# jordi-adell/mcarray

Hardware: AMD Instinct MI355X
Metric: STFT frames/sec, 8-mic GCC-PHAT + SRP-PHAT(361) + delay-and-sum beamform @48kHz/1024-pt (higher is better)
Workload: dtype f32 (SRP operands adaptive); 1 GPU; BASELINE configs[2] geometry (8-mic ULA 0.04 m, 48 kHz, N=1024, hop 512, 361 angles, 1 source, no power floor), 8 arrays x 4096 frames per GPU per step; channel rows padded by 64 floats; arrays_per_gpu=8, frames_per_array=4096, srp_precision=adaptive, parallelism=arrays sharded over 1 GPU(s), all_gather of DOA bins+prob

## Files before the change

### __graft_entry__.py

```python
import os
import subprocess
import sys

ROOT = os.path.dirname(os.path.abspath(__file__))
if ROOT not in sys.path:
    sys.path.insert(0, ROOT)


def build():
    env = dict(os.environ)
    subprocess.check_call(["make", "-C", os.path.join(ROOT, "mcarray_amd", "csrc"), "-j4", "-s"], env=env)
    subprocess.check_call(["make", "-C", os.path.join(ROOT, "oracle"), "-s"], env=env)
    cxx = os.path.join(ROOT, "tests", "cxx", "Makefile")
    if os.path.exists(cxx):
        subprocess.check_call(["make", "-C", os.path.dirname(cxx), "-s"], env=env)
    harness = os.path.join(ROOT, "tests", "cxx", "gemm_harness.mk")
    if os.path.exists(harness):
        subprocess.check_call(["make", "-C", os.path.dirname(harness), "-f", "gemm_harness.mk", "-s"], env=env)
    import mcarray_amd
    from mcarray_amd import _lib
    _lib.load()


def smoke():
    import numpy as np
    from mcarray_amd import api, synth
    from oracle import pyoracle as po
    fs, N, F = 48000, 1024, 12
    xs = synth.ULA8
    pcm = synth.noise_source_stream(xs, np.deg2rad(23.0), fs, (F + 1) * N // 2, 42)
    ctx = api.Context(fs, xs, N, 0.5, 1, srp_precision=api.SRP_FP32, device=0)
    r = ctx.process_frames_host(pcm[None], want_energy=True)
    o = po.ssl_stream(fs, N, xs, pcm.astype(np.float64), 1, 0.5, want_map=True)
    assert np.array_equal(r["bin"][0], o["bin"]), (r["bin"][0].T, o["bin"].T)
    assert np.abs(r["energy"][0] - o["energy"]).max() <= 2e-5 * np.abs(o["energy"]).max()
    assert np.abs(r["out"][0] - o["out"]).max() <= 2e-5 * np.abs(o["out"]).max() + 1e-7
    print("smoke ok: DOA bins", r["bin"][0, :, 0].tolist(), "->", float(np.rad2deg(r["doa"][0, -1, 0])), "deg")


if __name__ == "__main__":
    build()
    if len(sys.argv) > 1 and sys.argv[1] == "smoke":
        smoke()
```

### mcarray_amd/csrc/kernels_wave.hip

```cpp
#include <type_traits>

#include "fft1024c.h"
#include "mca_internal.h"
#include "cand_unit.h"
#include "phat_pairs.h"
#include "pair_balance.h"
#include "steer.h"
#include "stream_plan.h"

namespace mca {

__global__ __launch_bounds__(256) void k_bf_table(float2 *tab, const float *grid, const double *mic_x, int M, int n_pairs, double unit)
{
    const int d = blockIdx.x, pr = blockIdx.y;
    const double doa = d == 0 ? 0.0 : (double)grid[d - 1];
    const double cd = cos(doa + 1.57079632679489661923);
    const double sc = 1.0 / ((double)M * 1024.0);
    float2 *row = tab + ((long long)d * n_pairs + pr) * 1024;
    for (int k = threadIdx.x; k < 1024; k += 256) {
        const int kap = k <= 512 ? k : k - 1024;
        double pa[2] = {0.0, 0.0}, pb[2] = {0.0, 0.0};
        for (int e = 0; e < 2; ++e) {
            const int c = 2 * pr + e;
            if (c >= M) continue;
// ... 379 lines not shown
        auto load_pair = [&](int f, int pr) {
            const float *pa = base + (long long)(2 * pr) * mstride + (long long)(fr0 + f) * FFT_H;
            const float *pb = pa + mstride;
#pragma unroll
            for (int i = 0; i < 16; ++i) { xa[i] = pa[lofs + 64 * i]; xb[i] = pb[lofs + 64 * i]; }
        };
        const int nfr = f_end - f_begin;
        const int rot = p.list ? 0 : (int)((unsigned)(5 * a + 3 * ((int)blockIdx.x * nw + wave)) % (unsigned)nfr);
        auto frame_of = [&](int i) { const int j = i + rot; return f_begin + (j >= nfr ? j - nfr : j); };
        load_pair(frame_of(0), 0);
        const float4 *srow = nullptr; const float *snyq = nullptr;
        float2 *Yl = buf + F1K_SCRATCH + lam;
        float2 *Qs = wbase + nw * regw + wave * STEER_QWORDS;
        if (FUSE) {
            const int pred = __builtin_amdgcn_readfirstlane(p.bf.pred[a]) + 1;
            srow = p.bf.rows + (long long)pred * (NP * 64);
            snyq = p.bf.nyq + pred * MT;
            if (lane < STEER_QWORDS) Qs[lane] = p.bf.q[(pred * MT + 2 * (lane / 14) + (lane & 1)) * 8 + (lane % 14) / 2 + 1];
            wave_lds_fence();
        }
        for (int fi = 0; fi < nfr; ++fi) {
            const int f = frame_of(fi);
            float2 Xh[MT][8], zn[NP];
            float2 *yrow = FUSE ? p.bf.Y + ((long long)a * p.total_frames + p.frame0 + f) * STEER_ROW : nullptr;
            v2f ptime = {0.f, 0.f};
            bool any_alive = false;
#pragma unroll
            for (int pr = 0; pr < NP; ++pr) {
                float2 z[16];
                if (p.hist_out) {
                    const int j = p.frame0 + f - (p.total_frames - HIST_FRAMES);
                    if (j >= 0) {
                        float *ha = p.hist_out + ((long long)a * MT + 2 * pr) * HIST_SAMPLES + j * FFT_H + (FUSE ? 0 : lane);
#pragma unroll
                        for (int i = 0; i < 8; ++i) { ha[lofs + 64 * i] = xa[i]; ha[lofs + HIST_SAMPLES + 64 * i] = xb[i]; }
                        if (j == HIST_FRAMES - 1) {
#pragma unroll
                            for (int i = 0; i < 8; ++i) { ha[lofs + FFT_H + 64 * i] = xa[8 + i]; ha[lofs + HIST_SAMPLES + FFT_H + 64 * i] = xb[8 + i]; }
                        }
                    }
                }
#pragma unroll
                for (int i = 0; i < 8; ++i) { z[2 * i] = win_lo(xa[2 * i], xb[2 * i], win[i]); z[2 * i + 1] = win_hi(xa[2 * i + 1], xb[2 * i + 1], win[i]); }
                if (POWER) {
#pragma unroll
                    for (int i = 0; i < 16; ++i) { const v2f zv = to_v2f(z[i]); asm("v_pk_fma_f32 %0, %1, %1, %0" : "+v"(ptime) : "v"(zv)); }
                }
                float ma = max3abs(z[0].x, z[1].x, z[2].x), mb = max3abs(z[0].y, z[1].y, z[2].y);
#pragma unroll
                for (int i = 3; i < 15; i += 2) { ma = max3abs(ma, z[i].x, z[i + 1].x); mb = max3abs(mb, z[i].y, z[i + 1].y); }
                ma = max2abs(ma, z[15].x); mb = max2abs(mb, z[15].y);
                const PairBalance pb = pair_balance(ma, mb);
                const bool alive_a = pb.alive_a, alive_b = pb.alive_b;
                any_alive = any_alive || alive_a || alive_b;
                if (pb.scaled()) {
                    const float sa = pb.sa(), sb = pb.sb();
#pragma unroll
                    for (int i = 0; i < 16; ++i) z[i] = make_float2(z[i].x * sa, z[i].y * sb);
                }
                const float4 Bl = FUSE ? (srow + pr * 64)[(unsigned)lane] : make_float4(0.f, 0.f, 0.f, 0.f);
                fft1024c<false, 3>(z, buf, lane, tab, lc, [&]() {
                    const bool lastp = pr == NP - 1, last = lastp && fi + 1 >= nfr;
                    if (FUSE) { Yl[64 * STEER_Y_BASE] = make_float2(Bl.x, Bl.y); Yl[64 * (STEER_Y_BASE + 1)] = make_float2(Bl.z, Bl.w); }
                    load_pair(last ? f : (lastp ? frame_of(fi + 1) : f), last ? pr : (lastp ? 0 : pr + 1));
                }, lam);
                const float un_a = pb.un_a(), un_b = pb.un_b();
                if (MERGE && !FUSE) zn[pr] = make_float2(z[dr16(8)].x * un_a, z[dr16(8)].y * un_b);
                if (FUSE) { const float2 n = make_float2(z[dr16(8)].x * un_a, z[dr16(8)].y * un_b); if (pr < NP - 1) Yl[64 * (STEER_Y_ZN + pr)] = n; else zn[pr] = n; }
                if (lane == 0) {
                    const float2 n = z[dr16(8)];
                    if (!MERGE) nyq[(f - f_begin) * NP + pr] = make_float2(n.x * un_a, n.y * un_b);
                    float2 t[16];
#pragma unroll
                    for (int j = 0; j < 16; ++j) t[j] = z[dr16(j)];
#pragma unroll
                    for (int j = 8; j < 16; ++j) z[dr16(j < 12 ? j + 4 : j - 4)] = t[(j + 1) & 15];
                } else if (self) {
#pragma unroll
                    for (int j = 8; j < 12; ++j) { const float2 t = z[dr16(j)]; z[dr16(j)] = z[dr16(j + 4)]; z[dr16(j + 4)] = t; }
                } else {
#pragma unroll
                    for (int j = 8; j < 12; ++j) {
                        float2 &u = z[dr16(j)], &w = z[dr16(j + 4)];
                        swap_rows32(u.x, w.x); swap_rows32(w.x, u.x);
                        swap_rows32(u.y, w.y); swap_rows32(w.y, u.y);
                    }
                }
                const float thr_a = PairBalance::thr(4e-30f, pb.na, alive_a), thr_b = PairBalance::thr(4e-30f, pb.nb, alive_b);
                const float half_a = PairBalance::down(0.5f, pb.na, alive_a), half_b = PairBalance::down(0.5f, pb.nb, alive_b);
                float4 Bu = make_float4(0.f, 0.f, 0.f, 0.f);
                if (FUSE) { const float2 ba = Yl[64 * STEER_Y_BASE], bb = Yl[64 * (STEER_Y_BASE + 1)]; Bu = steer_base(make_float4(ba.x, ba.y, bb.x, bb.y), un_a, un_b); }
#pragma unroll
                for (int s = 0; s < 8; ++s) {
                    const float2 zk = z[dr16(s)], zm = z[dr16(15 - s < 12 ? 15 - s + 4 : 15 - s - 4)];
                    float2 a2, b2;
                    mirror_split(zk, zm, a2, b2);
                    if constexpr (ULA) whiten4_pair<NOPHAT>(a2, b2, Xh[2 * pr][s], Xh[2 * pr + 1][s], thr_a, thr_b, half_a, half_b);
                    else {
                        float pwa, pwb;
                        Xh[2 * pr][s] = whiten4<NOPHAT>(a2, pwa, thr_a, half_a);
                        Xh[2 * pr + 1][s] = whiten4<NOPHAT>(b2, pwb, thr_b, half_b);
                    }
                    if (FUSE) {
                        float2 y = pr == 0 ? make_float2(0.f, 0.f) : Yl[64 * s];
                        if (s == 0) y = steer_mac<true>(y, a2, b2, Bu, a2, b2);
                        else { const float4 qq = reinterpret_cast<const float4 *>(Qs)[pr * 7 + s - 1]; y = steer_mac<false>(y, a2, b2, Bu, make_float2(qq.x, qq.y), make_float2(qq.z, qq.w)); }
                        if (pr < NP - 1) Yl[64 * s] = y;
                        else yrow[(unsigned)lam + 64 * s] = s == 0 ? steer_dc(y, lane) : y;
                    }
                }
            }
            if (FUSE) {
#pragma unroll
                for (int pr = 0; pr < NP - 1; ++pr) zn[pr] = Yl[64 * (STEER_Y_ZN + pr)];
            }
            if (FUSE && lane == 0) yrow[FFT_H] = make_float2(steer_nyquist<NP>(zn, snyq), 0.f);
            if (p.dead && lane == 0) p.dead[(long long)a * p.total_frames + p.frame0 + f] = any_alive ? 0 : 1;
            OutT *arow = reinterpret_cast<OutT *>(p.A) + (row_base + f) * (long long)p.a_row_elems;
            if (MERGE) {
                float2 *S = buf;
                for (int j = lane; j < nmp / 2; j += 64) reinterpret_cast<float4 *>(S)[j] = make_float4(0.f, 0.f, 0.f, 0.f);
                wave_lds_fence();
                float xn[MT];
#pragma unroll
                for (int pr = 0; pr < NP; ++pr) {
                    float pw;
                    xn[2 * pr] = whiten4(make_float2(2.f * zn[pr].x, 0.f), pw).x;
                    xn[2 * pr + 1] = whiten4(make_float2(2.f * zn[pr].y, 0.f), pw).x;
                }
                const uint2 *offt = reinterpret_cast<const uint2 *>(rankl) + lane;
#pragma unroll
                for (int g = 1; g < MT; ++g) {
#pragma unroll
                    for (int h = 0; h < 2; ++h) {
                        const uint2 o4 = offt[(2 * (g - 1) + h) * 64];
                        const unsigned off[4] = {o4.x & 0xffffu, o4.x >> 16, o4.y & 0xffffu, o4.y >> 16};
                        float2 acc[4], cur[4];
#pragma unroll
                        for (int s2 = 0; s2 < 4; ++s2) {
                            acc[s2] = make_float2(0.f, 0.f);
#pragma unroll
                            for (int i = 0; i + g < MT; ++i) acc[s2] = cmacc(acc[s2], Xh[i][4 * h + s2], Xh[i + g][4 * h + s2]);
                        }
#pragma unroll
                        for (int s2 = 0; s2 < 4; ++s2) cur[s2] = S[off[s2]];
#pragma unroll
                        for (int s2 = 0; s2 < 4; ++s2) S[off[s2]] = cadd(cur[s2], acc[s2]);
                    }
                }
                if (lane == 0) {
                    float an[MT - 1], cn[MT - 1];
                    unsigned on[MT - 1];
#pragma unroll
                    for (int g = 1; g < MT; ++g) {
                        an[g - 1] = 0.f;
#pragma unroll
                        for (int i = 0; i + g < MT; ++i) an[g - 1] = fmaf(xn[i], xn[i + g], an[g - 1]);
                        on[g - 1] = rankl[2 * (MT - 1) * 64 * 4 + g - 1];
                    }
#pragma unroll
                    for (int g = 0; g < MT - 1; ++g) cn[g] = S[on[g]].x;
#pragma unroll
                    for (int g = 0; g < MT - 1; ++g) S[on[g]].x = cn[g] + an[g];
                }
                wave_lds_fence();
                typedef _Float16 half4_t __attribute__((ext_vector_type(4)));
                typedef float float4_t __attribute__((ext_vector_type(4)));
                if (p.planar) {
                    for (int j = lane; j < nmp / 4; j += 64) {
                        const float4 v0 = reinterpret_cast<const float4 *>(S)[2 * j], v1 = reinterpret_cast<const float4 *>(S)[2 * j + 1];
                        const float4_t re = {v0.x, v0.z, v1.x, v1.z}, im = {v0.y, v0.w, v1.y, v1.w};
                        reinterpret_cast<half4_t *>(arow)[j] = __builtin_convertvector(re, half4_t);
                        reinterpret_cast<half4_t *>(arow + nmp)[j] = __builtin_convertvector(im, half4_t);
                    }
                } else
                for (int j = lane; j < nmp / 2; j += 64) {
                    const float4 v = reinterpret_cast<const float4 *>(S)[j];
                    const float4_t vv = {v.x, v.y, v.z, v.w};
                    reinterpret_cast<half4_t *>(arow)[j] = __builtin_convertvector(vv, half4_t);
                }
                wave_lds_fence();
            } else {
#pragma unroll
                for (int s = 0; s < 8; ++s) {
                    if constexpr (ULA) {
                        float2 r[MT], out[NOUT];
#pragma unroll
                        for (int m = 0; m < MT; ++m) r[m] = Xh[m][s];
                        pair_products<MT, ULA>(r, out);
#pragma unroll
                        for (int g = 0; g < NOUT; ++g) store_a_wave<PL2>(arow, voff, g * KG + 64 * s, out[g], p.Kp);
                    } else {
                        int pi = 0;
#pragma unroll
                        for (int i = 0; i < MT; ++i)
#pragma unroll
                            for (int j = i + 1; j < MT; ++j) { store_a_wave<PL2>(arow, voff, pi * KG + 64 * s, cmulc(Xh[i][s], Xh[j][s]), p.Kp); ++pi; }
                    }
                }
            }
            if (POWER) {
                const float pacc = wave_sum64(ptime.x + ptime.y);
                if (lane == 0) p.power[(long long)a * p.total_frames + p.frame0 + f] = pacc / (float)FFT_N / (float)MT;
            }
        }
        wave_lds_fence();
        if (!MERGE && lane < f_end - f_begin) {
            float2 xn[MT], out[NOUT];
#pragma unroll
            for (int pr = 0; pr < NP; ++pr) {
                const float2 n = nyq[lane * NP + pr];
                float pw;
                xn[2 * pr] = whiten4<NOPHAT>(make_float2(2.f * n.x, 0.f), pw);
                xn[2 * pr + 1] = whiten4<NOPHAT>(make_float2(2.f * n.y, 0.f), pw);
            }
            OutT *arow = reinterpret_cast<OutT *>(p.A) + (row_base + f_begin + lane) * (long long)p.a_row_elems;
            pair_products<MT, ULA>(xn, out);
#pragma unroll
            for (int g = 0; g < NOUT; ++g) store_a_wave<PL2>(arow, 0u, g * KG + FFT_H, out[g], p.Kp);
        }
        }
        wave_lds_fence();
        if constexpr (CAND) {
            static_assert(!CAND || PL2, "the candidate contraction reads the two-plane rows of the list mode");
            {
                __syncthreads();
                cand_unit<4>(p.cand, li - p.list0, e_unit, reinterpret_cast<unsigned char *>(wbase), tid);
            }
        }
    }
}

__global__ __launch_bounds__(64) void k_steer_table(float4 *rows, float2 *q, float *nyq, const float *grid, const double *mic_x, int M, double unit)
{
    const int d = blockIdx.x, pr = blockIdx.y, lane = threadIdx.x, lam = lane <= 32 ? lane : 96 - lane;
    const double doa = d == 0 ? 0.0 : (double)grid[d - 1];
    const double cd = cos(doa + 1.57079632679489661923);
    const double sc = 1.0 / ((double)M * 1024.0);
    auto phasor = [&](int c, int k, double &cs, double &sn) {
        double turns = (double)k * (unit * mic_x[c] * cd);
        turns -= rint(turns);
        sincospi(2.0 * turns, &sn, &cs);
    };
    double ca, sa, cb, sb;
    phasor(2 * pr, lam, ca, sa); phasor(2 * pr + 1, lam, cb, sb);
    rows[((long long)d * gridDim.y + pr) * 64 + lane] = make_float4((float)(ca * sc), (float)(sa * sc), (float)(cb * sc), (float)(sb * sc));
    if (lane < 16) {
        const int c = 2 * pr + (lane >> 3), s = lane & 7;
        double cs, sn;
        phasor(c, 64 * s, cs, sn);
        q[((long long)d * M + c) * 8 + s] = make_float2((float)cs, (float)sn);
    }
    if (lane < 2) {
        double cs, sn;
        phasor(2 * pr + lane, 512, cs, sn);
        nyq[d * M + 2 * pr + lane] = (float)(cs * sc);
    }
}

__global__ __launch_bounds__(256, 2) void k_steer_patch(SteerPatchArgs p)
{
    extern __shared__ __attribute__((aligned(16))) unsigned char smem_raw[];
    float2 *tab = reinterpret_cast<float2 *>(smem_raw);
    const int tid = threadIdx.x, lane = tid & 63, wave = __builtin_amdgcn_readfirstlane(tid >> 6);
    float2 *buf = tab + F1K_TWORDS + wave * F1K_SCRATCH;
    const int npass = p.f1 - p.f0, stride = 4 * (int)gridDim.x;
    int work = p.all;
    if (!work) {
        const int first = (int)blockIdx.x * 4 + wave;
        const int per = first < npass ? (npass - first + stride - 1) / stride : 0, items = per * p.n_arrays;
        for (int i = lane; i < items; i += 64) {
            const int a = i / per, fo = first + stride * (i - a * per);
            work |= p.doa_bin[(long long)a * p.n_frames + p.f0 + fo] != p.bf.pred[a];
        }
    }
    if (!__syncthreads_or(work)) return;
    f1k_table_init(tab, tid, 256);
    F1kLane lc;
    lc.init(lane);
    __syncthreads();
    v2f win[8];
#pragma unroll
    for (int i = 0; i < 8; ++i) { win[i].x = p.window[lane + 128 * i]; win[i].y = p.window[lane + 128 * i + 64]; }
    for (int a = 0; a < p.n_arrays; ++a) {
        const int pred = __builtin_amdgcn_readfirstlane(p.bf.pred[a]);
        const bool every = p.all != 0;
        int missed = 0;
        for (int fo = (int)blockIdx.x * 4 + wave; fo < npass; fo += stride) {
            const int f = p.f0 + fo;
            const int bin = __builtin_amdgcn_readfirstlane(p.doa_bin[(long long)a * p.n_frames + f]);
            if (bin != pred) ++missed;
            else if (!every) continue;
            steer_patch_frame(p, a, f, bin, win, buf, tab, lc, lane);
        }
        if (missed && lane == 0) { atomicAdd(p.miss, (unsigned long long)missed); if (pred >= 0) atomicAdd(p.miss + 1, (unsigned long long)missed); }
    }
}

__global__ __launch_bounds__(256) void k_steer_synth(SteerSynthArgs p)
{
    extern __shared__ __attribute__((aligned(16))) unsigned char smem_raw[];
    float2 *tab = reinterpret_cast<float2 *>(smem_raw);
    const int tid = threadIdx.x, lane = tid & 63, wave = __builtin_amdgcn_readfirstlane(tid >> 6);
    float2 *buf = tab + F1K_TWORDS + wave * F1K_SCRATCH;
    f1k_table_init(tab, tid, 256);
    F1kLane lc;
    lc.init(lane);
    __syncthreads();
    const int a = blockIdx.y;
    if (p.pred_out && blockIdx.x == 0 && tid == 0) p.pred_out[a] = p.doa_bin[(long long)a * p.n_frames + p.n_frames - 1];
    if (p.report && blockIdx.x == 0 && a == 0 && tid == 0) {
        const unsigned long long tot = p.miss_total[1];
        p.report[0] = tot - p.miss_total[2];
        p.miss_total[2] = tot;
        __hip_atomic_store(&p.report[1], p.seq, __ATOMIC_RELEASE, __HIP_MEMORY_SCOPE_SYSTEM);
    }
    if (p.n_miss && blockIdx.x == 0 && a == 0 && tid == 0) *p.n_miss = 0;
    const int t0 = p.f0 + ((int)blockIdx.x * 4 + wave) * p.ft, t1 = min(t0 + p.ft, p.f1);
    if (t0 >= t1) return;
    const float2 *Yb = p.Y + ((long long)a * p.y_frames - p.y_f0) * STEER_ROW;
    float *ob = p.out + (long long)a * p.n_frames * FFT_H;
    float carry[8];
    if (t0 == p.f0) {
#pragma unroll
        for (int i = 0; i < 8; ++i) carry[i] = p.tail_in[(long long)a * FFT_H + lane + 64 * i];
    }
    int t = t0 > p.f0 ? t0 - 1 : t0;
    float2 yv[8], nv[8];
    float yn, nn = 0.f;
#pragma unroll
    for (int i = 0; i < 8; ++i) yv[i] = Yb[(long long)t * STEER_ROW + (unsigned)lane + 64 * i];
    yn = Yb[(long long)t * STEER_ROW + FFT_H].x;
    for (; t < t1; ++t) {
        float2 y[16];
        steer_inverse(y, yv, yn, buf, lane, tab, lc, [&]() {
            if (t + 1 < t1) {
#pragma unroll
                for (int i = 0; i < 8; ++i) nv[i] = Yb[(long long)(t + 1) * STEER_ROW + (unsigned)lane + 64 * i];
                nn = Yb[(long long)(t + 1) * STEER_ROW + FFT_H].x;
            }
        });
        if (t >= t0) {
#pragma unroll
            for (int i = 0; i < 8; ++i) ob[(long long)t * FFT_H + (unsigned)lane + 64 * i] = carry[i] + y[dr16(i)].x;
        }
#pragma unroll
        for (int i = 0; i < 8; ++i) { carry[i] = y[dr16(i + 8)].x; yv[i] = nv[i]; }
        yn = nn;
    }
    if (t1 == p.f1) {
#pragma unroll
        for (int i = 0; i < 8; ++i) p.tail_out[(long long)a * FFT_H + lane + 64 * i] = carry[i];
    }
}

typedef _Float16 h2 __attribute__((ext_vector_type(2)));
__device__ __forceinline__ h2 rot_j_conj(h2 b)
{
    h2 r;
    const unsigned c = 0x3C00BC00u;
    asm("v_pk_mul_f16 %0, %1, %2 op_sel:[1,0] op_sel_hi:[0,1]" : "=v"(r) : "v"(b), "v"(c));
    return r;
}

template <bool POWER>
__global__ __launch_bounds__(256, 2) void k_stft_phat_wave16(StftPhatArgs p)
{
    constexpr int MT = 16, NP = 8;
    extern __shared__ __attribute__((aligned(16))) unsigned char smem_raw[];
    float2 *tab = reinterpret_cast<float2 *>(smem_raw);
    const int tid = threadIdx.x, lane = tid & 63, wave = __builtin_amdgcn_readfirstlane(tid >> 6);
    float2 *buf = tab + F1K_TWORDS + wave * F1K_SCRATCH;
    float *wtab = reinterpret_cast<float *>(tab + F1K_TWORDS + 4 * F1K_SCRATCH);
    const int fpa = p.fpb + p.skew;
    float2 *nyq = reinterpret_cast<float2 *>(wtab + 1024) + wave * (fpa * NP);
    float2 *nref = reinterpret_cast<float2 *>(wtab + 1024) + 4 * (fpa * NP) + wave * (fpa * NP);
    float *dcbad = reinterpret_cast<float *>(reinterpret_cast<float2 *>(wtab + 1024) + 8 * (fpa * NP)) + wave * fpa;
    constexpr float UNSURE = 1e-10f;
    for (int e = tid; e < 1024; e += 256) wtab[(e & 63) * 16 + (e >> 6)] = p.window[e];
    f1k_table_init(tab, tid, 256);
    F1kLane lc;
    lc.init(lane);
    __syncthreads();
    const int lam = lane <= 32 ? lane : 96 - lane;
    const unsigned voff = (unsigned)lam * 4u;
    const bool self = (lane & 31) == 0;
    const float4 *wq = reinterpret_cast<const float4 *>(wtab + lane * 16);

    const int a = p.skew ? blockIdx.x : blockIdx.y;
    int f_begin = ((int)blockIdx.x * 4 + wave) * p.fpb, f_end = min(f_begin + p.fpb, p.n_frames);
    if (p.skew) {
        const int g = blockIdx.y, half = gridDim.y >> 1, hi = p.fpb + p.skew, lo = p.fpb - p.skew;
        if (g < half) { f_begin = (g * 4 + wave) * hi; f_end = f_begin + hi; }
        else { f_begin = half * 4 * hi + ((g - half) * 4 + wave) * lo; f_end = f_begin + lo; }
    }
    if (f_begin >= f_end) return;
    const long long row_base = (long long)a * p.n_frames;
    const float *base = p.pcm + (long long)a * p.array_stride + lane;
    float xa[16], xb[16];
    auto load_pair = [&](int f, int pr) {
        const float *pa = base + (long long)(2 * pr) * p.mic_stride + (long long)(p.frame0 + f) * FFT_H;
        const float *pb = pa + p.mic_stride;
#pragma unroll
        for (int i = 0; i < 16; ++i) { xa[i] = pa[64 * i]; xb[i] = pb[64 * i]; }
    };
    const int nfr = f_end - f_begin;
    const int rot = (int)((unsigned)(5 * a + 3 * ((int)blockIdx.x * 4 + wave)) % (unsigned)nfr);
    auto frame_of = [&](int i) { const int j = i + rot; return f_begin + (j >= nfr ? j - nfr : j); };
    load_pair(frame_of(0), 0);
    for (int fi = 0; fi < nfr; ++fi) {
        const int f = frame_of(fi);
        h2 Xh[MT][8];
        v2f ptime = {0.f, 0.f};
        bool dc_unsure = false;
#pragma unroll
        for (int pr = 0; pr < NP; ++pr) {
            float2 z[16];
#pragma unroll
            for (int i4 = 0; i4 < 4; ++i4) {
                const float4 w4 = wq[i4];
                const v2f w01 = {w4.x, w4.y}, w23 = {w4.z, w4.w};
                z[4 * i4] = win_lo(xa[4 * i4], xb[4 * i4], w01); z[4 * i4 + 1] = win_hi(xa[4 * i4 + 1], xb[4 * i4 + 1], w01);
                z[4 * i4 + 2] = win_lo(xa[4 * i4 + 2], xb[4 * i4 + 2], w23); z[4 * i4 + 3] = win_hi(xa[4 * i4 + 3], xb[4 * i4 + 3], w23);
            }
            float ref_a = 0.f, ref_b = 0.f;
            if (POWER || p.unsure) {
                v2f pz = {0.f, 0.f};
#pragma unroll
                for (int i = 0; i < 16; ++i) { const v2f zv = to_v2f(z[i]); asm("v_pk_fma_f32 %0, %1, %1, %0" : "+v"(pz) : "v"(zv)); }
                if (POWER) { ptime.x += pz.x; ptime.y += pz.y; }
                if (p.unsure) { ref_a = 4.f * wave_sum64(pz.x); ref_b = 4.f * wave_sum64(pz.y); }
            }
            float ma = max3abs(z[0].x, z[1].x, z[2].x), mb = max3abs(z[0].y, z[1].y, z[2].y);
#pragma unroll
            for (int i = 3; i < 15; i += 2) { ma = max3abs(ma, z[i].x, z[i + 1].x); mb = max3abs(mb, z[i].y, z[i + 1].y); }
            ma = max2abs(ma, z[15].x); mb = max2abs(mb, z[15].y);
            const PairBalance pb = pair_balance(ma, mb);
            const bool alive_a = pb.alive_a, alive_b = pb.alive_b;
            float dc_a = ref_a, dc_b = ref_b;
            if (pb.scaled()) {
                const float sa = pb.sa(), sb = pb.sb();
#pragma unroll
                for (int i = 0; i < 16; ++i) z[i] = make_float2(z[i].x * sa, z[i].y * sb);
                dc_a *= sa * sa; dc_b *= sb * sb;
            }
            fft1024c<false, 3>(z, buf, lane, tab, lc, [&]() {
                const bool lastp = pr == NP - 1, last = lastp && fi + 1 >= nfr;
                load_pair(last ? f : (lastp ? frame_of(fi + 1) : f), last ? pr : (lastp ? 0 : pr + 1));
            }, lam);
            if (lane == 0) {
                const float2 n = z[dr16(8)];
                nyq[(f - f_begin) * NP + pr] = make_float2(n.x * pb.un_a(), n.y * pb.un_b());
                float2 t[16];
#pragma unroll
                for (int j = 0; j < 16; ++j) t[j] = z[dr16(j)];
#pragma unroll
                for (int j = 8; j < 16; ++j) z[dr16(j < 12 ? j + 4 : j - 4)] = t[(j + 1) & 15];
            } else if (self) {
#pragma unroll
                for (int j = 8; j < 12; ++j) { const float2 t = z[dr16(j)]; z[dr16(j)] = z[dr16(j + 4)]; z[dr16(j + 4)] = t; }
            } else {
#pragma unroll
                for (int j = 8; j < 12; ++j) {
                    float2 &u = z[dr16(j)], &w = z[dr16(j + 4)];
                    swap_rows32(u.x, w.x); swap_rows32(w.x, u.x);
                    swap_rows32(u.y, w.y); swap_rows32(w.y, u.y);
                }
            }
            float pw0a = 0.f, pw0b = 0.f;
            const float thr_a = PairBalance::thr(4e-30f, pb.na, alive_a), thr_b = PairBalance::thr(4e-30f, pb.nb, alive_b);
#pragma unroll
            for (int s = 0; s < 8; ++s) {
                const float2 zk = z[dr16(s)], zm = z[dr16(15 - s < 12 ? 15 - s + 4 : 15 - s - 4)];
                const float2 a2 = make_float2(zk.x + zm.x, zk.y - zm.y);
                const float2 b2 = make_float2(zk.y + zm.y, zm.x - zk.x);
                float pwa, pwb;
                const float2 wa = whiten4<false>(a2, pwa, thr_a), wb = whiten4<false>(b2, pwb, thr_b);
                const float2_t va = {wa.x, wa.y}, vb = {wb.x, wb.y};
                Xh[2 * pr][s] = __builtin_convertvector(va, h2);
                Xh[2 * pr + 1][s] = __builtin_convertvector(vb, h2);
                if (s == 0) { pw0a = pwa; pw0b = pwb; }
                if (s == 0 && p.unsure && lane == 0) {
                    nref[(f - f_begin) * NP + pr] = make_float2(ref_a, ref_b);
                    dc_unsure = dc_unsure || (pw0a < UNSURE * dc_a) || (pw0b < UNSURE * dc_b);
                }
            }
        }
        if (p.unsure && lane == 0) dcbad[f - f_begin] = dc_unsure ? 1.f : 0.f;
        _Float16 *arow = reinterpret_cast<_Float16 *>(p.A) + (row_base + f) * (long long)p.a_row_elems;
#pragma unroll
        for (int s = 0; s < 8; ++s) {
            __builtin_amdgcn_sched_barrier(0);
            h2 rj[MT];
#pragma unroll
            for (int j = 1; j < MT; ++j) rj[j] = rot_j_conj(Xh[j][s]);
            float re[MT - 1], im[MT - 1];
#pragma unroll
            for (int g = 0; g < MT - 1; ++g) { re[g] = 0.f; im[g] = 0.f; }
#pragma unroll
            for (int i = 0; i < MT; ++i)
#pragma unroll
                for (int j = i + 1; j < MT; ++j) {
                    re[j - i - 1] = __builtin_amdgcn_fdot2(Xh[i][s], Xh[j][s], re[j - i - 1], false);
                    im[j - i - 1] = __builtin_amdgcn_fdot2(Xh[i][s], rj[j], im[j - i - 1], false);
                }
#pragma unroll
            for (int g = 0; g < MT - 1; ++g) store_a_wave<false>(arow, voff, g * KG + 64 * s, make_float2(re[g], im[g]), p.Kp);
        }
        if (POWER) {
            const float pacc = wave_sum64(ptime.x + ptime.y);
            if (lane == 0) p.power[(long long)a * p.total_frames + p.frame0 + f] = pacc / (float)FFT_N / (float)MT;
        }
    }
    wave_lds_fence();
    if (lane < f_end - f_begin) {
        float2 xn[MT], out[MT - 1];
#pragma unroll
        for (int pr = 0; pr < NP; ++pr) {
            const float2 n = nyq[lane * NP + pr];
            float pw;
            xn[2 * pr] = whiten4<false>(make_float2(2.f * n.x, 0.f), pw);
            xn[2 * pr + 1] = whiten4<false>(make_float2(2.f * n.y, 0.f), pw);
        }
        if (p.unsure) {
            bool u = dcbad[lane] != 0.f;
#pragma unroll
            for (int pr = 0; pr < NP; ++pr) {
                const float2 n = nyq[lane * NP + pr], r = nref[lane * NP + pr];
                u = u || (4.f * n.x * n.x < UNSURE * r.x) || (4.f * n.y * n.y < UNSURE * r.y);
            }
            p.unsure[(long long)a * p.total_frames + p.frame0 + f_begin + lane] = u ? 1 : 0;
        }
        _Float16 *arow = reinterpret_cast<_Float16 *>(p.A) + (row_base + f_begin + lane) * (long long)p.a_row_elems;
        pair_products<MT, true>(xn, out);
#pragma unroll
        for (int g = 0; g < MT - 1; ++g) store_a_wave<false>(arow, 0u, g * KG + FFT_H, out[g], p.Kp);
    }
}
const void *stft_wave16_kernel(const StftForm &f)
{
    return f.power ? reinterpret_cast<const void *>(&k_stft_phat_wave16<true>) : reinterpret_cast<const void *>(&k_stft_phat_wave16<false>);
}

const void *stft_wave_kernel(const StftForm &f)
{
    const void *kernel = nullptr;
    plan_static_for<2 << 8>([&](auto rc) {
        constexpr int r = decltype(rc)::value, MT = r & 1 ? 8 : 4;
        constexpr bool ULA = r & 2, F32 = r & 4, PL2 = r & 8, POWER = r & 16, NOPHAT = r & 32, MERGE = r & 64, CAND = r & 128, FUSE = r & 256;
        if constexpr (stft_wave_row(MT, ULA, F32, PL2, POWER, NOPHAT, MERGE, CAND, FUSE)) {
            using T = std::conditional_t<F32, float, _Float16>;
            if (f.mt == MT && f.ula == ULA && f.f32 == F32 && f.pl2 == PL2 && f.power == POWER && f.nophat == NOPHAT && f.merge == MERGE && f.cand == CAND && f.fuse == FUSE)
                kernel = reinterpret_cast<const void *>(&k_stft_phat_wave<MT, ULA, T, PL2, POWER, NOPHAT, MERGE, CAND, FUSE>);
        }
    });
    return kernel;
}

}
```

### mcarray_amd/csrc/steer.h

```cpp
#pragma once
#include "fft1024c.h"
#include "mca_internal.h"
#include "pair_balance.h"

namespace mca {

__device__ __forceinline__ float4 steer_base(float4 B, float un_a, float un_b)
{
    const float2 a = cscale(make_float2(B.x, B.y), un_a), b = cscale(make_float2(B.z, B.w), un_b);
    return make_float4(a.x, a.y, b.x, b.y);
}
template <bool FIRST>
__device__ __forceinline__ float2 steer_mac(float2 y, float2 a2, float2 b2, float4 B, float2 qa, float2 qb)
{
    if (!FIRST) { a2 = cmul(a2, qa); b2 = cmul(b2, qb); }
    y = cmac(y, a2, make_float2(B.x, B.y));
    return cmac(y, b2, make_float2(B.z, B.w));
}
__device__ __forceinline__ float2 steer_dc(float2 y0, int lane) { return cscale(y0, lane == 0 ? 0.5f : 1.f); }

template <int NP>
__device__ __forceinline__ float steer_nyquist(const float2 (&zn)[NP], const float *pn)
{
    float yn = 0.f;
#pragma unroll
    for (int pr = 0; pr < NP; ++pr) yn = fmaf(zn[pr].y, pn[2 * pr + 1], fmaf(zn[pr].x, pn[2 * pr], yn));
    return yn;
}

template <typename Mid = F1kNoMid>
__device__ __forceinline__ void steer_inverse(float2 (&y)[16], const float2 (&yv)[8], float yn, float2 *buf, int lane, const float2 *tab, const F1kLane &lc, Mid mid = Mid())
{
#pragma unroll
    for (int i = 0; i < 8; ++i) { y[i] = yv[i]; y[i + 8] = make_float2(0.f, 0.f); }
    fft1024c<true, 3>(y, buf, lane, tab, lc, mid);
    const float sn = (lane & 1) ? -yn : yn;
#pragma unroll
    for (int i = 0; i < 16; ++i) y[i].x += sn;
}

__device__ __forceinline__ float2 win_lo(float a, float b, v2f w)
{
    v2f x = {a, b}, r;
    asm("v_pk_mul_f32 %0, %1, %2 op_sel:[0,0] op_sel_hi:[1,0]" : "=v"(r) : "v"(x), "v"(w));
    return from_v2f(r);
}
__device__ __forceinline__ float2 win_hi(float a, float b, v2f w)
{
    v2f x = {a, b}, r;
    asm("v_pk_mul_f32 %0, %2, %1 op_sel:[1,0] op_sel_hi:[1,1]" : "=v"(r) : "v"(x), "v"(w));
    return from_v2f(r);
}

__device__ __forceinline__ void mirror_split(float2 zk, float2 zm, float2 &a2, float2 &b2)
{
    const v2f k = to_v2f(zk), m = to_v2f(zm);
    v2f a, b;
    asm("v_pk_add_f32 %0, %1, %2 neg_hi:[0,1]" : "=v"(a) : "v"(k), "v"(m));
    asm("v_pk_fma_f32 %0, %1, 1.0, %2 op_sel:[1,0,1] op_sel_hi:[0,0,0] neg_hi:[1,0,0]" : "=v"(b) : "v"(k), "v"(m));
    a2 = from_v2f(a);
    b2 = from_v2f(b);
}

__device__ __forceinline__ void steer_patch_frame(const SteerPatchArgs &p, int a, int f, int bin, const v2f (&win)[8], float2 *buf, const float2 *tab,
                                                  const F1kLane &lc, int lane)
{
    constexpr int NP = 4, MT = 8;
    const int lam = lane <= 32 ? lane : 96 - lane;
    const bool self = (lane & 31) == 0;
    const float4 *srow = p.bf.rows + (long long)(bin + 1) * (NP * 64);
    const float2 *qrow = p.bf.q + (long long)(bin + 1) * (MT * 8);
    const float *base = p.pcm + (long long)a * p.array_stride + (long long)f * FFT_H;
    float2 *yrow = p.bf.Y + ((long long)a * p.y_frames + f - p.y_f0) * STEER_ROW;
    float xa[16], xb[16];
    auto load_pair = [&](int pr) {
        const float *pa = base + (long long)(2 * pr) * p.mic_stride, *pb = pa + p.mic_stride;
#pragma unroll
        for (int i = 0; i < 16; ++i) { xa[i] = pa[(unsigned)lane + 64 * i]; xb[i] = pb[(unsigned)lane + 64 * i]; }
    };
    load_pair(0);
    float2 Y[8], zn[NP];
#pragma unroll
    for (int pr = 0; pr < NP; ++pr) {
        float2 z[16];
        float4 B;
#pragma unroll
        for (int i = 0; i < 8; ++i) { z[2 * i] = win_lo(xa[2 * i], xb[2 * i], win[i]); z[2 * i + 1] = win_hi(xa[2 * i + 1], xb[2 * i + 1], win[i]); }
        float ma = max3abs(z[0].x, z[1].x, z[2].x), mb = max3abs(z[0].y, z[1].y, z[2].y);
#pragma unroll
        for (int i = 3; i < 15; i += 2) { ma = max3abs(ma, z[i].x, z[i + 1].x); mb = max3abs(mb, z[i].y, z[i + 1].y); }
        ma = max2abs(ma, z[15].x); mb = max2abs(mb, z[15].y);
        const PairBalance pb = pair_balance(ma, mb);
        if (pb.scaled()) {
            const float sa = pb.sa(), sb = pb.sb();
#pragma unroll
            for (int i = 0; i < 16; ++i) z[i] = make_float2(z[i].x * sa, z[i].y * sb);
        }
        fft1024c<false, 3>(z, buf, lane, tab, lc, [&]() {
            B = (srow + pr * 64)[(unsigned)lane];
            if (pr < NP - 1) load_pair(pr + 1);
        }, lam);
        const float un_a = pb.un_a(), un_b = pb.un_b();
        zn[pr] = make_float2(z[dr16(8)].x * un_a, z[dr16(8)].y * un_b);
        const float4 Bu = steer_base(B, un_a, un_b);
        if (lane == 0) {
            float2 t[16];
#pragma unroll
            for (int j = 0; j < 16; ++j) t[j] = z[dr16(j)];
#pragma unroll
            for (int j = 8; j < 16; ++j) z[dr16(j < 12 ? j + 4 : j - 4)] = t[(j + 1) & 15];
        } else if (self) {
#pragma unroll
            for (int j = 8; j < 12; ++j) { const float2 t = z[dr16(j)]; z[dr16(j)] = z[dr16(j + 4)]; z[dr16(j + 4)] = t; }
        } else {
#pragma unroll
            for (int j = 8; j < 12; ++j) {
                float2 &u = z[dr16(j)], &w = z[dr16(j + 4)];
                swap_rows32(u.x, w.x); swap_rows32(w.x, u.x);
                swap_rows32(u.y, w.y); swap_rows32(w.y, u.y);
            }
        }
#pragma unroll
        for (int s = 0; s < 8; ++s) {
            const float2 zk = z[dr16(s)], zm = z[dr16(15 - s < 12 ? 15 - s + 4 : 15 - s - 4)];
            const float2 a2 = make_float2(zk.x + zm.x, zk.y - zm.y);
            const float2 b2 = make_float2(zk.y + zm.y, zm.x - zk.x);
            const float2 y = pr == 0 ? make_float2(0.f, 0.f) : Y[s];
            if (s == 0) Y[s] = steer_mac<true>(y, a2, b2, Bu, a2, b2);
            else Y[s] = steer_mac<false>(y, a2, b2, Bu, qrow[(2 * pr) * 8 + s], qrow[(2 * pr + 1) * 8 + s]);
        }
        wave_lds_fence();
    }
#pragma unroll
    for (int s = 0; s < 8; ++s) yrow[(unsigned)lam + 64 * s] = s == 0 ? steer_dc(Y[s], lane) : Y[s];
    if (lane == 0) yrow[FFT_H] = make_float2(steer_nyquist<NP>(zn, p.bf.nyq + (bin + 1) * MT), 0.f);
}

}
```

Baseline: 59.95 million frames/s.

## Use half-length complex inverse FFT for real-output steer synthesis

Replaces the full 1024-point complex inverse FFT in the steer-synthesis kernel with a 512-point complex inverse FFT plus a real-signal split/pack step, which exploits the Hermitian symmetry of the beamformed spectrum. Output and overlap-add carry are now handled as packed float2 pairs written with 8-byte vector stores. The aim is to roughly halve the FFT arithmetic and LDS traffic per synthesized frame. The cost is extra lane-swap shuffles and more complex index bookkeeping, plus dependence on new table helpers (FftTw, TW_WIN, fft_table_init) that are not visible in the prior code.

```diff
diff --git a/__graft_entry__.py b/__graft_entry__.py
--- a/__graft_entry__.py
+++ b/__graft_entry__.py
@@ -17,6 +17,9 @@
     harness = os.path.join(ROOT, "tests", "cxx", "gemm_harness.mk")
     if os.path.exists(harness):
         subprocess.check_call(["make", "-C", os.path.dirname(harness), "-f", "gemm_harness.mk", "-s"], env=env)
+    harness = os.path.join(ROOT, "tests", "cxx", "steer_harness.mk")
+    if os.path.exists(harness):
+        subprocess.check_call(["make", "-C", os.path.dirname(harness), "-f", "steer_harness.mk", "-s"], env=env)
     import mcarray_amd
     from mcarray_amd import _lib
     _lib.load()
diff --git a/mcarray_amd/csrc/kernels_wave.hip b/mcarray_amd/csrc/kernels_wave.hip
--- a/mcarray_amd/csrc/kernels_wave.hip
+++ b/mcarray_amd/csrc/kernels_wave.hip
@@ -705,11 +705,12 @@
     extern __shared__ __attribute__((aligned(16))) unsigned char smem_raw[];
     float2 *tab = reinterpret_cast<float2 *>(smem_raw);
     const int tid = threadIdx.x, lane = tid & 63, wave = __builtin_amdgcn_readfirstlane(tid >> 6);
-    float2 *buf = tab + F1K_TWORDS + wave * F1K_SCRATCH;
-    f1k_table_init(tab, tid, 256);
-    F1kLane lc;
-    lc.init(lane);
+    float2 *buf = tab + TW_WIN + wave * FFT_SCRATCH;
+    fft_table_init(tab, nullptr, tid, 256);
+    const FftTw tw{tab};
     __syncthreads();
+    SteerHalfLane hl;
+    hl.init(lane, tw);
     const int a = blockIdx.y;
     if (p.pred_out && blockIdx.x == 0 && tid == 0) p.pred_out[a] = p.doa_bin[(long long)a * p.n_frames + p.n_frames - 1];
     if (p.report && blockIdx.x == 0 && a == 0 && tid == 0) {
@@ -723,37 +724,40 @@
     if (t0 >= t1) return;
     const float2 *Yb = p.Y + ((long long)a * p.y_frames - p.y_f0) * STEER_ROW;
     float *ob = p.out + (long long)a * p.n_frames * FFT_H;
-    float carry[8];
+    typedef v2f __attribute__((aligned(4))) v2f_u;
+    const unsigned m2 = 2u * (unsigned)hl.lam;
+    float2 carry[4];
     if (t0 == p.f0) {
 #pragma unroll
-        for (int i = 0; i < 8; ++i) carry[i] = p.tail_in[(long long)a * FFT_H + lane + 64 * i];
+        for (int j = 0; j < 4; ++j) carry[j] = from_v2f(*reinterpret_cast<const v2f_u *>(p.tail_in + (long long)a * FFT_H + m2 + 128 * j));
     }
     int t = t0 > p.f0 ? t0 - 1 : t0;
-    float2 yv[8], nv[8];
-    float yn, nn = 0.f;
-#pragma unroll
-    for (int i = 0; i < 8; ++i) yv[i] = Yb[(long long)t * STEER_ROW + (unsigned)lane + 64 * i];
-    yn = Yb[(long long)t * STEER_ROW + FFT_H].x;
+    float2 yv[8], nv[8], y256, n256 = make_float2(0.f, 0.f);
+#pragma unroll
+    for (int i = 0; i < 8; ++i) yv[i] = Yb[(long long)t * STEER_ROW + (unsigned)(i < 4 ? hl.lam : hl.lamx) + 64 * i];
+    y256 = Yb[(long long)t * STEER_ROW + FFT_H / 2];
     for (; t < t1; ++t) {
-        float2 y[16];
-        steer_inverse(y, yv, yn, buf, lane, tab, lc, [&]() {
+        steer_inverse_half(yv, y256, buf, lane, tw, hl, [&]() {
             if (t + 1 < t1) {
 #pragma unroll
-                for (int i = 0; i < 8; ++i) nv[i] = Yb[(long long)(t + 1) * STEER_ROW + (unsigned)lane + 64 * i];
-                nn = Yb[(long long)(t + 1) * STEER_ROW + FFT_H].x;
+                for (int i = 0; i < 8; ++i) nv[i] = Yb[(long long)(t + 1) * STEER_ROW + (unsigned)(i < 4 ? hl.lam : hl.lamx) + 64 * i];
+                n256 = Yb[(long long)(t + 1) * STEER_ROW + FFT_H / 2];
             }
         });
         if (t >= t0) {
 #pragma unroll
-            for (int i = 0; i < 8; ++i) ob[(long long)t * FFT_H + (unsigned)lane + 64 * i] = carry[i] + y[dr16(i)].x;
-        }
-#pragma unroll
-        for (int i = 0; i < 8; ++i) { carry[i] = y[dr16(i + 8)].x; yv[i] = nv[i]; }
-        yn = nn;
+            for (int j = 0; j < 4; ++j)
+                *reinterpret_cast<v2f_u *>(ob + (long long)t * FFT_H + m2 + 128 * j) = to_v2f(cadd(carry[j], yv[br3(j)]));
+        }
+#pragma unroll
+        for (int j = 0; j < 4; ++j) carry[j] = yv[br3(j + 4)];
+#pragma unroll
+        for (int i = 0; i < 8; ++i) yv[i] = nv[i];
+        y256 = n256;
     }
     if (t1 == p.f1) {
 #pragma unroll
-        for (int i = 0; i < 8; ++i) p.tail_out[(long long)a * FFT_H + lane + 64 * i] = carry[i];
+        for (int j = 0; j < 4; ++j) *reinterpret_cast<v2f_u *>(p.tail_out + (long long)a * FFT_H + m2 + 128 * j) = to_v2f(carry[j]);
     }
 }
 
diff --git a/mcarray_amd/csrc/steer.h b/mcarray_amd/csrc/steer.h
--- a/mcarray_amd/csrc/steer.h
+++ b/mcarray_amd/csrc/steer.h
@@ -37,6 +37,111 @@
     const float sn = (lane & 1) ? -yn : yn;
 #pragma unroll
     for (int i = 0; i < 16; ++i) y[i].x += sn;
+}
+
+struct SteerHalfLane {
+    float2 wh[4];
+    float2 dc;
+    int lam, lamx;
+    __device__ __forceinline__ void init(int lane, const FftTw &tw)
+    {
+        lam = lane <= 32 ? lane : 96 - lane;
+        lamx = lane == 0 ? 32 : lane == 32 ? 64 : lam;
+        dc = lane == 0 ? make_float2(2.f, 0.f) : make_float2(1.f, 1.f);
+#pragma unroll
+        for (int s = 0; s < 4; ++s) wh[s] = tw.ts(s, lam);
+    }
+};
+
+__device__ __forceinline__ void swap_lanes32(float2 &u, float2 &w)
+{
+    swap_rows32(u.x, w.x); swap_rows32(w.x, u.x);
+    swap_rows32(u.y, w.y); swap_rows32(w.y, u.y);
+}
+
+__device__ __forceinline__ float2 steer_pk_mul(float2 x, v2f c)
+{
+    v2f r;
+    asm("v_pk_mul_f32 %0, %1, %2" : "=v"(r) : "v"(to_v2f(x)), "v"(c));
+    return from_v2f(r);
+}
+__device__ __forceinline__ void steer_split_pair(float2 ak, float2 ap, float2 w, float2 &zk, float2 &zp)
+{
+    const v2f cj = {1.f, -1.f}, hh = {0.5f, 0.5f}, hj = {0.5f, -0.5f};
+    const float2 cp = steer_pk_mul(ap, cj);
+    const float2 a = cadd(ak, cp), b = cmulc(csub(ak, cp), w);
+    zk = steer_pk_mul(cadd_jb(a, b), hh);
+    zp = steer_pk_mul(csub_jb(a, b), hj);
+}
+
+__device__ __forceinline__ void fft8_inv_pk(float2 (&v)[8])
+{
+    constexpr float R = 0.70710678118654752440f;
+#pragma unroll
+    for (int r = 0; r < 4; ++r) {
+        const float2 a = cadd(v[r], v[r + 4]), b = csub(v[r], v[r + 4]);
+        v[r] = a;
+        v[r + 4] = r == 0 ? b : r == 1 ? cscale(cadd_jb(b, b), R) : r == 2 ? cmul_pj(b) : cscale(csub_jb(b, b), -R);
+    }
+#pragma unroll
+    for (int h = 0; h < 8; h += 4) {
+        bfly4<true>(v[h], v[h + 1], v[h + 2], v[h + 3]);
+        const float2 t = v[h + 1]; v[h + 1] = v[h + 2]; v[h + 2] = t;
+    }
+}
+
+template <typename Mid>
+__device__ __forceinline__ void cfft512_inv_pk(float2 (&v)[8], float2 *buf, int lane, const FftTw &tw, Mid mid)
+{
+    float2 twa[8], twb[8];
+#pragma unroll
+    for (int i = 1; i < 8; ++i) twa[i] = tw.t1(br3(i), lane);
+    fft8_inv_pk(v);
+#pragma unroll
+    for (int i = 0; i < 8; ++i) buf[br3(i) * FFT_ROW + lane] = i == 0 ? v[i] : cmulc(v[i], twa[i]);
+    wave_lds_fence();
+    mid();
+    const int qq = lane >> 3, l0 = lane & 7;
+#pragma unroll
+    for (int l1 = 0; l1 < 8; ++l1) v[l1] = buf[qq * FFT_ROW + l0 + 8 * l1];
+    wave_lds_fence();
+#pragma unroll
+    for (int i = 1; i < 8; ++i) twb[i] = tw.t2(br3(i), lane);
+    fft8_inv_pk(v);
+#pragma unroll
+    for (int i = 0; i < 8; ++i) buf[qq + 66 * l0 + 8 * br3(i)] = i == 0 ? v[i] : cmulc(v[i], twb[i]);
+    wave_lds_fence();
+#pragma unroll
+    for (int j = 0; j < 8; ++j) v[j] = buf[lane + 66 * j];
+    wave_lds_fence();
+    fft8_inv_pk(v);
+}
+
+template <typename Mid = F1kNoMid>
+__device__ __forceinline__ void steer_inverse_half(float2 (&v)[8], float2 a256, float2 *buf, int lane, const FftTw &tw, const SteerHalfLane &hl, Mid mid = Mid())
+{
+    swap_lanes32(v[4], v[7]);
+    swap_lanes32(v[5], v[6]);
+    {
+        const v2f dc = to_v2f(hl.dc);
+        v2f a0 = to_v2f(v[0]), an = to_v2f(v[4]);
+        asm("v_pk_mul_f32 %0, %1, %2" : "=v"(a0) : "v"(a0), "v"(dc));
+        asm("v_pk_mul_f32 %0, %1, %2" : "=v"(an) : "v"(an), "v"(dc));
+        v[0] = from_v2f(a0); v[4] = from_v2f(an);
+    }
+#pragma unroll
+    for (int s = 0; s < 4; ++s) steer_split_pair(v[s], v[4 + s], hl.wh[s], v[s], v[4 + s]);
+    if ((lane & 31) != 0) {
+        swap_lanes32(v[4], v[7]);
+        swap_lanes32(v[5], v[6]);
+    } else if (lane == 0) {
+        const float2 t = v[5];
+        v[4] = cconj(a256); v[5] = v[7]; v[7] = t;
+    } else {
+        float2 t = v[4]; v[4] = v[7]; v[7] = t;
+        t = v[5]; v[5] = v[6]; v[6] = t;
+    }
+    cfft512_inv_pk(v, buf, hl.lam, tw, mid);
 }
 
 __device__ __forceinline__ float2 win_lo(float a, float b, v2f w)
```

New measurement: 60.47 million frames/s, median of 6. About the same (+0.9%).
